# CobayaSampler/cobaya

Measured on AMD Instinct MI355X. Metric: log-posterior evals/sec (whole node), 30-dim gaussian_mixture, higher is better.
Workload: dtype f64

## Files before the change

cobaya_amd/csrc/capi.hip:

```cpp
#include "ctx.h"
#include "host_linalg.h"

int block_slots(const mcmc_hip_ctx* h, int which)
{
    if (!h->blocked) return h->d;
    int L = 0;
    for (size_t b = 0; b < h->blk_size.size(); ++b) {
        if (which == 0) L += h->blk_over[b] * h->blk_size[b];
        else if (which == 1) L += ((int)b <= h->drag_last_slow) ? h->blk_size[b] : 0;
        else L += ((int)b > h->drag_last_slow) ? h->blk_size[b] : 0;
    }
    return L;
}

int upload_constants(mcmc_hip_ctx* h)
{
    if (!h->have_prior || !h->have_target) return MCMC_HIP_OK;
    const int d = h->d, K = h->K;
    const ConstLayout cl{d, K};
    std::vector<double> c((size_t)cl.size() + 16, 0.0);
    for (int i = 0; i < d; ++i) {
        c[cl.lo() + i] = h->lo[i];
        c[cl.hi() + i] = h->hi[i];
        c[cl.loc() + i] = h->loc[i];
// ... 86 lines not shown
        return fail(h, MCMC_HIP_ERR_ARG,
                    "the step kernel needs %zu bytes of LDS per workgroup (> 160 KiB): fewer "
                    "mixture modes or a smaller group_size are required", lds);
    return MCMC_HIP_OK;
}

int set_target_common(mcmc_hip_ctx* h, int K, const double* means, const double* covs,
                      const double* weights, bool normalized)
{
    const int d = h->d;
    if (K < 1 || K > mcmc::kMaxModes)
        return fail(h, MCMC_HIP_ERR_ARG, "n_modes must be in 1..%d, got %d", mcmc::kMaxModes, K);
    if (h->huge && K > mcmc::kHugeMaxModes)
        return fail(h, MCMC_HIP_ERR_ARG, "d=%d > %d serves at most %d mixture modes, got %d", d, kMaxDimBig,
                    mcmc::kHugeMaxModes, K);
    std::vector<double> L((size_t)d * d), Li((size_t)d * d);
    h->mean.assign(means, means + (size_t)K * d);
    h->Linv.assign((size_t)K * d * d, 0.0);
    h->cnorm.assign(K, 0.0);
    h->weight.assign(K, 1.0 / K);
    for (int k = 0; k < K; ++k) {
        const double* C = covs + (size_t)k * d * d;
        if (!is_symmetric(d, C) || !cholesky_lower(d, C, L.data()))
            return fail(h, MCMC_HIP_ERR_NOT_PD,
                        "covariance of mode %d is not a symmetric positive-definite matrix", k);
        tri_inverse_lower(d, L.data(), Li.data());
        std::copy(Li.begin(), Li.end(), h->Linv.begin() + (size_t)k * d * d);
        double logdet = 0.0;
        for (int i = 0; i < d; ++i) logdet += std::log(L[i * d + i]);
        logdet *= 2.0;
        h->cnorm[k] = normalized ? d * std::log(2.0 * M_PI) + logdet : 0.0;
    }
    if (weights) {
        double s = 0.0;
        for (int k = 0; k < K; ++k) {
            if (!(weights[k] >= 0.0)) return fail(h, MCMC_HIP_ERR_ARG, "negative mixture weight");
            s += weights[k];
        }
        if (!(s > 0.0)) return fail(h, MCMC_HIP_ERR_ARG, "mixture weights sum to zero");
        const bool renorm = !(std::fabs(s - 1.0) <= 1e-8 + 1e-5);
        for (int k = 0; k < K; ++k) h->weight[k] = renorm ? weights[k] / s : weights[k];
    }
    h->K = K;
    h->bg.on = false;
    h->fnt.on = false;
    h->have_target = true;
    ++h->dir_epoch;
    h->have_state = false;
    int rc = lds_check(h);
    if (rc) return rc;
    return upload_constants(h);
}

}

extern "C" {

const char* mcmc_hip_version(void) { return "mcmc_hip 0.1 (gfx950)"; }

const char* mcmc_hip_last_error(const mcmc_hip_ctx* h)
{
    return h ? h->err.c_str() : g_create_error.c_str();
}

int mcmc_hip_dim_supported(int d)
{
    return kernels_for_dim(d) != nullptr || big_for_dim(d) != nullptr;
}

int32_t mcmc_hip_max_dim(void) { return mcmc::kMaxDimHuge; }

int mcmc_hip_create(const mcmc_hip_config* cfg, mcmc_hip_ctx** out)
{
    if (!cfg || !out) return fail(nullptr, MCMC_HIP_ERR_ARG, "null argument");
    *out = nullptr;
    if (cfg->d < 1) return fail(nullptr, MCMC_HIP_ERR_ARG, "d must be >= 1, got %d", cfg->d);
    const DimKernels* k = kernels_for_dim(cfg->d);
    const BigKernels* kb = k ? nullptr : big_for_dim(cfg->d);
    const bool huge = cfg->d > kMaxDimBig;
    if (huge) {
        if (cfg->d > mcmc::kMaxDimHuge)
            return fail(nullptr, MCMC_HIP_ERR_ARG, "d=%d is above the largest dimension served (%d)",
                        cfg->d, mcmc::kMaxDimHuge);
        if (!(cfg->flags & MCMC_HIP_FLAG_INCREMENTAL))
            return fail(nullptr, MCMC_HIP_ERR_ARG,
                        "d=%d > %d is served with incremental evaluation only (evaluation: full is not)",
                        cfg->d, kMaxDimBig);
        if (cfg->flags & MCMC_HIP_FLAG_OWN_BASIS)
            return fail(nullptr, MCMC_HIP_ERR_ARG, "d=%d > %d needs the shared basis (shared_basis: False is not served)",
                        cfg->d, kMaxDimBig);
        if (cfg->emit_capacity > 0)
            return fail(nullptr, MCMC_HIP_ERR_ARG,
                        "d=%d > %d emits no rows on the device (emit: chains is not served; use emit: snapshots)",
                        cfg->d, kMaxDimBig);
    }
    if (!k && !kb && !huge)
        return fail(nullptr, MCMC_HIP_ERR_ARG,
                    "no kernels compiled for d=%d (this build covers d = 1..32 lane-per-walker "
                    "and 33..%d column-sweep, as selected at build time)", cfg->d, kMaxDimBig);
    if (cfg->group_size != 64 && cfg->group_size != 128 && cfg->group_size != 256)
        return fail(nullptr, MCMC_HIP_ERR_ARG, "group_size must be 64, 128 or 256, got %d",
                    cfg->group_size);
    if (cfg->n_walkers < cfg->group_size || cfg->n_walkers % cfg->group_size)
        return fail(nullptr, MCMC_HIP_ERR_ARG,
                    "n_walkers (%d) must be a positive multiple of group_size (%d)",
                    cfg->n_walkers, cfg->group_size);
// ... 25 lines not shown
    int ndev = 0;
    hipError_t e = hipGetDeviceCount(&ndev);
    if (e != hipSuccess || ndev <= 0)
        return fail(nullptr, MCMC_HIP_ERR_DEVICE, "no HIP device available (%s)",
                    e == hipSuccess ? "device count 0" : hipGetErrorString(e));
    if (cfg->device < 0 || cfg->device >= ndev)
        return fail(nullptr, MCMC_HIP_ERR_ARG, "device %d out of range (0..%d)", cfg->device,
                    ndev - 1);
    hipDeviceProp_t prop;
    if (hipGetDeviceProperties(&prop, cfg->device) != hipSuccess)
        return fail(nullptr, MCMC_HIP_ERR_DEVICE, "hipGetDeviceProperties failed");
    if (std::strncmp(prop.gcnArchName, "gfx950", 6) != 0)
        return fail(nullptr, MCMC_HIP_ERR_DEVICE,
                    "device %d is %s; this library is built for gfx950 only", cfg->device,
                    prop.gcnArchName);
    if (hipSetDevice(cfg->device) != hipSuccess)
        return fail(nullptr, MCMC_HIP_ERR_DEVICE, "hipSetDevice(%d) failed", cfg->device);
    mcmc_hip_ctx* h = new mcmc_hip_ctx();
    h->cfg = *cfg;
    h->k = k;
    h->kb = kb;
    h->huge = huge;
    h->kp = (kb && !getenv("MCMC_HIP_NO_PAIR_BIG")) ? pair_for_dim(cfg->d) : nullptr;
    h->d = cfg->d;
    h->W = cfg->n_walkers;
    h->gs = cfg->group_size;
    h->G = h->W / h->gs;
    h->bgs = h->gs << ((cfg->flags & MCMC_HIP_FLAG_BASIS_GROUP_MASK) >> 8);
    h->BG = h->W / h->bgs;
    h->shift.assign(h->d, 0.0);
    h->incremental = (cfg->flags & MCMC_HIP_FLAG_INCREMENTAL) != 0;
    h->own_basis = (cfg->flags & MCMC_HIP_FLAG_OWN_BASIS) != 0 && cfg->d > 1;
    if (hipStreamCreateWithFlags(&h->stream, hipStreamNonBlocking) != hipSuccess) {
        delete h;
        return fail(nullptr, MCMC_HIP_ERR_DEVICE, "hipStreamCreate failed");
    }
    const size_t W = h->W, d = h->d, G = h->G, np = d * (d + 1) / 2;
    hipError_t r = hipSuccess;
    auto acc = [&](hipError_t x) { if (r == hipSuccess) r = x; };
    acc(h->x.resize(W * d)); acc(h->logpost.resize(W)); acc(h->logprior.resize(W));
    acc(h->loglike.resize(W)); acc(h->weight_i.resize(W)); acc(h->prej.resize(W));
    acc(h->burn.resize(W)); acc(h->nacc.resize(W)); acc(h->stuck.resize(1));
    acc(h->dT.resize(d * d + 16));  acc(h->Sg.resize(G * np));
    acc(h->gsum.resize(G * d + np + 1));
    if (r == hipSuccess) {
        h->pooled.p = h->gsum.p + G * d;
        h->acc_total.p = reinterpret_cast<unsigned long long*>(h->gsum.p + G * d + np);
    }
    acc(h->dshift.resize(d));
    if (cfg->emit_capacity > 0) {
        acc(h->rows.resize(W * (size_t)cfg->emit_capacity * (d + 4)));
        acc(h->nrows.resize(W));
    }
    acc(hipHostMalloc((void**)&h->pin_mom, sizeof(double) * (G * d + np + 2), hipHostMallocDefault));
    acc(hipHostMalloc((void**)&h->pin_T, sizeof(double) * 4 * d * d, hipHostMallocDefault));
    for (auto& e : h->pin_T_done) acc(hipEventCreateWithFlags(&e, hipEventDisableTiming));
    acc(hipEventCreateWithFlags(&h->mom_event, hipEventDisableTiming));
    if (h->incremental) {
        int prio_least = 0, prio_greatest = 0;
        acc(hipDeviceGetStreamPriorityRange(&prio_least, &prio_greatest));
        acc(hipStreamCreateWithPriority(&h->stream2, hipStreamNonBlocking, prio_least));
        acc(hipEventCreateWithFlags(&h->mark, hipEventDisableTiming));
        acc(hipEventCreateWithFlags(&h->T_event, hipEventDisableTiming));
        if (const char* e = getenv("MCMC_HIP_EAGER_DIRECTIONS")) h->lazy_dirs = !(e[0] && e[0] != '0');
        if (const char* e = getenv("MCMC_HIP_LOOKAHEAD")) h->lookahead = std::max(1, atoi(e));
        if (const char* e = getenv("MCMC_HIP_DUO")) h->duo = (e[0] && e[0] != '0') ? 1 : 0;
        if (const char* e = getenv("MCMC_HIP_ACCEPT_SLACK")) {
            const double v = strtod(e, nullptr);
            h->accept_slack = v < mcmc::kAcceptSlack ? mcmc::kAcceptSlack : v;
        }
        for (auto& D : h->dirs) acc(hipEventCreateWithFlags(&D.ready, hipEventDisableTiming));
        h->prefetch = !getenv("MCMC_HIP_NO_PREFETCH");
    }
    if (r == hipSuccess) r = hipMemsetAsync(h->gsum.p, 0, sizeof(double) * G * d, h->stream);
    if (r == hipSuccess) r = hipMemsetAsync(h->pooled.p, 0, sizeof(double) * np, h->stream);
    if (r == hipSuccess) r = hipMemsetAsync(h->dshift.p, 0, sizeof(double) * d, h->stream);
    if (r == hipSuccess) r = hipMemsetAsync(h->stuck.p, 0, sizeof(int), h->stream);
    if (r == hipSuccess) r = hipMemsetAsync(h->acc_total.p, 0, sizeof(unsigned long long), h->stream);
    if (r == hipSuccess) r = hipStreamSynchronize(h->stream);
    if (r != hipSuccess) {
        fail(nullptr, MCMC_HIP_ERR_DEVICE, "device allocation failed: %s", hipGetErrorString(r));
        mcmc_hip_destroy(h);
        return MCMC_HIP_ERR_DEVICE;
    }
    *out = h;
    return MCMC_HIP_OK;
}

void mcmc_hip_destroy(mcmc_hip_ctx* h)
{
    if (!h) return;
    (void)hipSetDevice(h->cfg.device);
    if (h->stream) (void)hipStreamSynchronize(h->stream);
    if (h->stream2) (void)hipStreamSynchronize(h->stream2);
    resolve_timing(h);
    for (auto e : h->pool) (void)hipEventDestroy(e);
    for (auto& D : h->dirs) {
        D.V.release(); D.Vf.release(); D.VU.release(); D.vflag.release(); D.vflag_f.release(); D.UU.release();
        D.colflag.release(); D.VW.release(); D.NL.release();
        if (D.ready) (void)hipEventDestroy(D.ready);
    }
    if (h->mark) (void)hipEventDestroy(h->mark);
    if (h->T_event) (void)hipEventDestroy(h->T_event);
    if (h->stream2) (void)hipStreamDestroy(h->stream2);
    h->x.release(); h->logpost.release(); h->logprior.release(); h->loglike.release();
    h->hV.release(); h->hScratch.release(); h->hCols.release();
    h->cblock.release(); h->dT.release(); h->V.release(); h->rows.release(); h->gsum.release();
// ... 705 lines not shown
}

int mcmc_hip_read_moments(mcmc_hip_ctx* h, int64_t* n_snapshots, double* group_sum,
                          double* pooled_S, int32_t reset)
{
    if (!h) return MCMC_HIP_ERR_ARG;
    HIP_TRY(h, hipSetDevice(h->cfg.device));
    HIP_TRY(h, hipStreamSynchronize(h->stream));
    if (h->stream2) HIP_TRY(h, hipStreamSynchronize(h->stream2));
    resolve_timing(h);
    const size_t d = h->d, G = h->G, np = d * (d + 1) / 2;
    if (n_snapshots) *n_snapshots = h->n_snapshots;
    if (group_sum)
        HIP_TRY(h, hipMemcpy(group_sum, h->gsum.p, sizeof(double) * G * d, hipMemcpyDeviceToHost));
    if (pooled_S) {
        std::vector<double> p(np);
        HIP_TRY(h, hipMemcpy(p.data(), h->pooled.p, sizeof(double) * np, hipMemcpyDeviceToHost));
        for (size_t i = 0; i < d; ++i)
            for (size_t j = 0; j <= i; ++j)
                pooled_S[i * d + j] = pooled_S[j * d + i] = p[i * (i + 1) / 2 + j];
    }
    if (reset) {
        HIP_TRY(h, hipMemset(h->gsum.p, 0, sizeof(double) * G * d));
        HIP_TRY(h, hipMemset(h->pooled.p, 0, sizeof(double) * np));
        h->n_snapshots = 0;
    }
    return MCMC_HIP_OK;
}

int mcmc_hip_set_moments(mcmc_hip_ctx* h, int64_t n_snapshots, const double* group_sum,
                         const double* pooled_S)
{
    if (!h || !group_sum || !pooled_S || n_snapshots < 0) return MCMC_HIP_ERR_ARG;
    HIP_TRY(h, hipSetDevice(h->cfg.device));
    HIP_TRY(h, hipStreamSynchronize(h->stream));
    const size_t d = h->d, G = h->G, np = d * (d + 1) / 2;
    std::vector<double> p(np);
    for (size_t i = 0; i < d; ++i)
        for (size_t j = 0; j <= i; ++j) p[i * (i + 1) / 2 + j] = pooled_S[i * d + j];
    HIP_TRY(h, hipMemcpy(h->gsum.p, group_sum, sizeof(double) * G * d, hipMemcpyHostToDevice));
    HIP_TRY(h, hipMemcpy(h->pooled.p, p.data(), sizeof(double) * np, hipMemcpyHostToDevice));
    h->n_snapshots = n_snapshots;
    return MCMC_HIP_OK;
}

int mcmc_hip_request_moments(mcmc_hip_ctx* h)
{
    if (!h) return MCMC_HIP_ERR_ARG;
    if (!h->have_state) return fail(h, MCMC_HIP_ERR_STATE, "no state");
    if (h->mom_pending) return fail(h, MCMC_HIP_ERR_STATE, "a moment request is already pending");
    HIP_TRY(h, hipSetDevice(h->cfg.device));
    const size_t d = h->d, G = h->G, np = d * (d + 1) / 2;
    hipStream_t s = h->stream;
    HIP_TRY(h, hipMemcpyAsync(h->pin_mom, h->gsum.p, sizeof(double) * (G * d + np + 1),
                              hipMemcpyDeviceToHost, s));
    HIP_TRY(h, hipMemcpyAsync(h->pin_mom + G * d + np + 1, h->stuck.p, sizeof(int),
                              hipMemcpyDeviceToHost, s));
    if (h->fnt.on)
        HIP_TRY(h, hipMemcpyAsync(reinterpret_cast<int*>(h->pin_mom + G * d + np + 1) + 1, h->fnt.bad.p,
                                  sizeof(int), hipMemcpyDeviceToHost, s));
    h->mom_fn = h->fnt.on;
    if (!h->ck.ring.p) HIP_TRY(h, hipMemsetAsync(h->gsum.p, 0, sizeof(double) * (G * d + np), s));
    HIP_TRY(h, hipEventRecord(h->mom_event, s));
    h->mom_n = h->n_snapshots;
    h->mom_step = h->step;
    h->n_snapshots = 0;
    h->mom_pending = true;
    return MCMC_HIP_OK;
}

int mcmc_hip_fetch_moments(mcmc_hip_ctx* h, int64_t* n_snapshots, double* group_sum,
                           double* pooled_S, int64_t counters[2])
{
    if (!h) return MCMC_HIP_ERR_ARG;
    if (!h->mom_pending) return fail(h, MCMC_HIP_ERR_STATE, "no moment request is pending");
    HIP_TRY(h, hipSetDevice(h->cfg.device));
    HIP_TRY(h, hipEventSynchronize(h->mom_event));
    h->mom_pending = false;
    const size_t d = h->d, G = h->G, np = d * (d + 1) / 2;
    if (n_snapshots) *n_snapshots = h->mom_n;
    if (group_sum) std::copy(h->pin_mom, h->pin_mom + G * d, group_sum);
    if (pooled_S) {
        const double* p = h->pin_mom + G * d;
        for (size_t i = 0; i < d; ++i)
            for (size_t j = 0; j <= i; ++j)
                pooled_S[i * d + j] = pooled_S[j * d + i] = p[i * (i + 1) / 2 + j];
    }
    if (counters) {
        unsigned long long tot;
        std::memcpy(&tot, h->pin_mom + G * d + np, sizeof tot);
        counters[0] = (int64_t)h->mom_step;
        counters[1] = (int64_t)tot;
    }
    if (h->mom_fn) {
        int bad = 0;
        std::memcpy(&bad, reinterpret_cast<const int*>(h->pin_mom + G * d + np + 1) + 1, sizeof bad);
        if (bad) return function_target_error(h, bad);
    }
    int stuck = 0;
    std::memcpy(&stuck, h->pin_mom + G * d + np + 1, sizeof stuck);
    if (stuck)
        return fail(h, MCMC_HIP_ERR_STUCK,
                    "The chain has been stuck for %g attempts (walker %d), stopping sampling.",
                    h->cfg.max_tries, stuck - 1);
    return MCMC_HIP_OK;
}

void mcmc_hip_note_step_kernel(const char* name) { g_noted_kernel = name; }

const char* mcmc_hip_last_step_kernel(const mcmc_hip_ctx* h)
{
    return h ? h->last_step_kernel.c_str() : "";
}

int mcmc_hip_enable_timing(mcmc_hip_ctx* h, int32_t on)
// ... 42 lines not shown
```

cobaya_amd/csrc/ctx.h:

```cpp
#pragma once
#include "../../include/mcmc_hip.h"

#include <algorithm>
#include <cmath>
#include <cstdarg>
#include <cstdio>
#include <cstring>
#include <limits>
#include <string>
#include <vector>

#define MCMC_HIP_HOST_SIDE 1
#include "kernels.h"
#include "huge_args.h"
#include "pliklite_args.h"
#include "function_args.h"
#include "checkpoint_args.h"
#include "marginal_args.h"
#include "autocorr_args.h"
#include "bestfit_args.h"
#include "evidence_args.h"
#include "derived_args.h"
#include "comm.h"
#include "inc_choice.h"
// ... 103 lines not shown
    unsigned long long hV_cycle = ~0ull, hV_epoch = ~0ull;
    hipStream_t stream = nullptr;
    std::string err;
    int d = 0, W = 0, G = 0, gs = 0, K = -1;
    bool have_prior = false, have_target = false, have_cov = false, have_state = false;
    std::vector<int32_t> kind, periodic;
    std::vector<double> lo, hi, loc, scale, mls;
    double uniform_logp = 0.0;
    uint32_t norm_mask = 0, periodic_mask = 0;
    uint32_t norm_mask4[4] = {0, 0, 0, 0};
    bool any_periodic = false;
    std::vector<double> mean, Linv, cnorm, weight;
    std::vector<double> cov, T;
    bool blocked = false;
    std::vector<int32_t> blk_size, blk_over, i_of_j;
    int drag_last_slow = -1, drag_steps = 0;
    DevBuf<int> dblk, vflag, vflag_f;
    DevBuf<double> Vf;
    DevBuf<double> drag_cs;
    std::vector<double> shift;
    DevBuf<double> x, logpost, logprior, loglike, cblock, dT, V, rows, gsum, Sg, pooled, dshift;
    DevBuf<double> ex, elp, ell, eder, escratch, dLrow, dLcol;
    bool incremental = false;
    bool y_valid = false;
    bool own_basis = false;
    int bgs = 0, BG = 0;
    DevBuf<double> y, inc_prior, inc_Lrow, inc_mean;
    DevBuf<double> amode;
    bool amode_valid = false;
    struct DirSet {
        DevBuf<double> V, Vf, VU;
        DevBuf<int> vflag, vflag_f, colflag;
        bool has_flags = false;
        DevBuf<double> UU;
        DevBuf<double> VW, NL;
        hipEvent_t ready = nullptr;
        bool ahead = false;
        unsigned long long step0 = ~0ull, epoch = 0;
        int n = 0;
    } dirs[2];
    int dir_cur = 0;
    unsigned long long dir_epoch = 0;
    hipStream_t stream2 = nullptr;
    hipEvent_t mark = nullptr;
    bool mark_valid = false;
    bool prefetch = true;
    bool lazy_dirs = true;
    int lookahead = 4;
    int duo = -1;
    double accept_slack = mcmc::kAcceptSlack;
    hipEvent_t T_event = nullptr;
    bool T_fresh = false;
    double* pin_mom = nullptr;
    double* pin_T = nullptr;
    int pin_T_slot = 0;
    hipEvent_t pin_T_done[4] = {nullptr, nullptr, nullptr, nullptr};
    hipEvent_t mom_event = nullptr;
    bool mom_pending = false;
    bool mom_fn = false;
    int64_t mom_n = 0;
    unsigned long long mom_step = 0;
    struct HostSlot { double* p = nullptr; size_t cap_rows = 0; };
    std::vector<HostSlot> slots = std::vector<HostSlot>(4);
    int slot_next = 0;
    DevBuf<double> pack_out;
    DevBuf<long long> pack_off;
    DevBuf<int> weight_i, prej, burn, stuck, nrows;
    DevBuf<int> thin_acc;
    int emit_thin = 1;
    DevBuf<long long> nacc;
    DevBuf<unsigned long long> acc_total;
    unsigned long long step = 0;
    int64_t n_snapshots = 0;
    bool timing = false;
    struct Ev {
        hipEvent_t a, b;
        int kind;
    };
    std::vector<Ev> pending;
    std::vector<hipEvent_t> pool;
    double ms[6] = {0, 0, 0, 0, 0, 0};
    int64_t n_seen[6] = {0, 0, 0, 0, 0, 0}, n_timed[6] = {0, 0, 0, 0, 0, 0};
    int64_t n_step_launches = 0;
    std::string last_step_kernel;
    struct Ckpt {
        DevBuf<double> ring, wsum, payload, ws, out;
        DevBuf<unsigned long long> acc_prev;
        int cap = 0;
        long long n_done = 0;
        double* pin_out = nullptr;
        hipEvent_t ev = nullptr;
        bool begun = false, pending = false;
        bool payload_only = false;
    } ck;
    struct Bounds {
        DevBuf<double> ring, bounds, payload;
        int n_slots = 0;
        double* pin = nullptr;
    } bd;
    struct Marginals {
        DevBuf<unsigned long long> slab;
        DevBuf<mcmc::MargEntry> entries;
        unsigned long long* pin = nullptr;
        size_t n_counters = 0, off_pairs = 0;
        int n1 = 0, n2 = 0, bins1 = 0, bins2 = 0, n_entries = 0, lds_words = 0;
        int64_t n_acc = 0;
// ... 177 lines not shown
```

cobaya_amd/csrc/incremental_kernels.hip:

```cpp
#include <string>

#include "incremental_common.h"

#ifndef MCMC_INC_DMA_HIDDEN
#define MCMC_INC_DMA_HIDDEN(dq, mode) ((dq) >= 25 && (mode) == 0)
#endif

namespace mcmc {
namespace {

__host__ __device__ constexpr bool inc_one_wave_regs(int dq, int mode, bool per)
{
    return !per && ((mode == 1 && dq >= 31) || (mode == 2 && dq >= 32));
}

__host__ __device__ constexpr int inc_min_waves(int dq, int mode, bool per = false)
{
    if (per) return MCMC_EXP_WAVES(STEP, dq <= 8 ? 4 : dq <= 31 ? 2 : 1);
    return MCMC_EXP_WAVES(STEP,
        mode == 0 ? (dq <= 12 ? 4 : dq <= 30 ? 2 : 1)
        : mode == 1 ? ((dq <= 8 || dq == 13) ? 4 : dq <= 30 ? 2 : 1)
        : (dq <= 8 ? 4 : dq <= 31 ? 2 : 1));
}

// ... 812 lines not shown
                            const pair_t p = col2[4 * kk];
                            const double delta = ra * p.x;
                            cs[kk] = cs[kk] + delta;
                            ce[kk] = ce[kk] + delta;
                            ys[kk] = fma(ra, p.y, ys[kk]);
                            ye[kk] = fma(ra, p.y, ye[kk]);
                        }
                        cs_lt = sel(acc_m, ps_lt, cs_lt);
                        ce_lp = sel(acc_m, pe_lp, ce_lp);
                        ce_ll = sel(acc_m, pe_ll, ce_ll);
                        ce_lt = sel(acc_m, pe_lt, ce_lt);
                        start_acc += cs_lt;
                        end_acc += ce_lt;
                    }
                }
            }
            const unsigned long long accept_m =
                ~lanes(dead) & metropolis(end_acc / navg, start_acc / navg, Ea0);
            const bool accept = __builtin_amdgcn_inverse_ballot_w64(accept_m);
            const int lim = burn > 0 ? lim10 : lim1;
            burn -= (accept & (burn > 0)) ? 1 : 0;
            lpri = sel(accept_m, ce_lp, lpri);
            llik = sel(accept_m, ce_ll, llik);
            lpost = sel(accept_m, ce_lt, lpost);
            prej = sel(accept_m, 0, prej);
            wt = sel(accept_m, 1, wt + 1);
            nacc += sel(accept_m, 1, 0);
            if (!accept & !dead & (wt - prej > lim) && c == 0) atomicCAS(s.stuck, 0, 1 + (int)gid);
#pragma unroll
            for (int kk = 0; kk < DQ; ++kk) {
                x0[kk] = sel(accept_m, ce[kk], x0[kk]);
                y0[kk] = sel(accept_m, ye[kk], y0[kk]);
            }
        }
        asm volatile("s_waitcnt vmcnt(0)" ::: "memory");
        __syncthreads();
    }
#pragma unroll
    for (int kk = 0; kk < DQ; ++kk) {
        const int i = 4 * kk + c;
        if (i < d) {
            s.x[(size_t)i * W + w] = x0[kk];
            a.y[(size_t)i * W + w] = y0[kk];
        }
    }
    if (c == 0) {
        s.logpost[w] = lpost; s.logprior[w] = lpri; s.loglike[w] = llik;
        s.weight[w] = wt; s.prior_rej[w] = prej; s.burn_left[w] = burn;
        s.n_accept[w] = nacc;
    }
    wave_add_accepts(s.accept_total, (c == 0) ? nacc - nacc0 : 0);
}

__global__ void __launch_bounds__(256) whiten_state_kernel(const double* __restrict__ x,
                                                           double* __restrict__ y,
                                                           const double* __restrict__ mean,
                                                           const double* __restrict__ Lrow, int d,
                                                           int W, int K)
{
    extern __shared__ __attribute__((aligned(16))) double sdev[];
    const int l = threadIdx.x & 63, part = __builtin_amdgcn_readfirstlane(threadIdx.x >> 6),
              w = blockIdx.x * 64 + l;
    const bool live = w < W;
    const int nblk = (d + 3) / 4;
    for (int k = 0; k < K; ++k) {
        __syncthreads();
        if (live)
            for (int i = part; i < d; i += 4) sdev[i * 64 + l] = x[(size_t)i * W + w] - mean[k * d + i];
        __syncthreads();
        if (!live) continue;
        for (int rb = part; rb < nblk; rb += 4) {
            const int j0 = 4 * rb;
            if (j0 + 4 <= d) {
                const double* __restrict__ r0 = Lrow + ((size_t)k * d + j0) * d;
                const double* __restrict__ r1 = r0 + d;
                const double* __restrict__ r2 = r1 + d;
                const double* __restrict__ r3 = r2 + d;
                double a0 = 0.0, a1 = 0.0, a2 = 0.0, a3 = 0.0;
                for (int i = 0; i <= j0; ++i) {
                    const double dv = sdev[i * 64 + l];
                    a0 = fma(r0[i], dv, a0);
                    a1 = fma(r1[i], dv, a1);
                    a2 = fma(r2[i], dv, a2);
                    a3 = fma(r3[i], dv, a3);
                }
                const double d1 = sdev[(j0 + 1) * 64 + l], d2 = sdev[(j0 + 2) * 64 + l],
                             d3 = sdev[(j0 + 3) * 64 + l];
                a1 = fma(r1[j0 + 1], d1, a1);
                a2 = fma(r2[j0 + 1], d1, a2);
                a3 = fma(r3[j0 + 1], d1, a3);
                a2 = fma(r2[j0 + 2], d2, a2);
                a3 = fma(r3[j0 + 2], d2, a3);
                a3 = fma(r3[j0 + 3], d3, a3);
                double* __restrict__ out = y + ((size_t)k * d + j0) * W + w;
                out[0] = a0; out[(size_t)W] = a1; out[2 * (size_t)W] = a2; out[3 * (size_t)W] = a3;
            } else {
                for (int j = j0; j < d; ++j) {
                    const double* __restrict__ row = Lrow + ((size_t)k * d + j) * d;
                    double acc = 0.0;
                    for (int i = 0; i <= j; ++i) acc = fma(row[i], sdev[i * 64 + l], acc);
                    y[((size_t)k * d + j) * W + w] = acc;
                }
            }
        }
    }
}

__global__ void __launch_bounds__(256) whiten_directions_kernel(const IncDirArgs a)
{
    extern __shared__ __attribute__((aligned(16))) double sv[];
    const int l = threadIdx.x & 63, part = __builtin_amdgcn_readfirstlane(threadIdx.x >> 6);
    const int sr = blockIdx.x * 64 + l;
    const int g = blockIdx.y;
    const int d = a.d;
    const bool live = sr < a.n_steps;
    int flag1d = 0;
    if (live) {
        const unsigned long long step = a.step0 + (unsigned long long)sr;
        const int cyc = (int)(step / (unsigned long long)a.cps - a.cycle0);
        const int col = (int)(step % (unsigned long long)a.cps);
        const double* __restrict__ v = a.V + ((size_t)g * a.ncyc + cyc) * a.slab + (size_t)col * a.ld;
        for (int i = part; i < d; i += 4) sv[i * 64 + l] = v[i];
        if (a.vflag) flag1d = a.vflag[((size_t)g * a.ncyc + cyc) * a.cps + col];
    }
    __syncthreads();
    if (!live) return;
    const size_t ocol = a.out_div ? (size_t)(sr / a.out_div) * a.out_cols + a.out_slot0 + sr % a.out_div
                                  : (size_t)sr;
    double2* __restrict__ out = (double2*)a.VU + ((size_t)g * a.out_total + ocol) * (4 * a.dq);
    if (a.colflag && part == 0) a.colflag[(size_t)g * a.out_total + ocol] = flag1d;
    const int nblk = (d + 3) / 4;
    for (int rb = part; rb < nblk; rb += 4) {
        const int j = 4 * rb;
        if (j + 4 <= d) {
            const cdoubles r0 = (cdoubles)(unsigned long long)(a.Lrow + (size_t)j * d);
            const cdoubles r1 = r0 + d;
            const cdoubles r2 = r1 + d;
            const cdoubles r3 = r2 + d;
            double a0 = 0.0, a1 = 0.0, a2 = 0.0, a3 = 0.0;
            for (int i = 0; i <= j; ++i) {
                const double v = sv[i * 64 + l];
                a0 = fma(r0[i], v, a0);
                a1 = fma(r1[i], v, a1);
                a2 = fma(r2[i], v, a2);
                a3 = fma(r3[i], v, a3);
            }
            const double v1 = sv[(j + 1) * 64 + l], v2 = sv[(j + 2) * 64 + l], v3 = sv[(j + 3) * 64 + l];
            a1 = fma(r1[j + 1], v1, a1);
            a2 = fma(r2[j + 1], v1, a2);
            a3 = fma(r3[j + 1], v1, a3);
            a2 = fma(r2[j + 2], v2, a2);
            a3 = fma(r3[j + 2], v2, a3);
            a3 = fma(r3[j + 3], v3, a3);
            out[j] = make_double2(sv[j * 64 + l], a0);
            out[j + 1] = make_double2(v1, a1);
            out[j + 2] = make_double2(v2, a2);
            out[j + 3] = make_double2(v3, a3);
        } else {
            for (int jj = j; jj < d; ++jj) {
                const cdoubles row = (cdoubles)(unsigned long long)(a.Lrow + (size_t)jj * d);
                double acc = 0.0;
                for (int i = 0; i <= jj; ++i) acc = fma(row[i], sv[i * 64 + l], acc);
                out[jj] = make_double2(sv[jj * 64 + l], acc);
            }
        }
    }
    if (part == 3)
        for (int j = d; j < 4 * a.dq; ++j) out[j] = make_double2(0.0, 0.0);
    if (a.UU) {
        __shared__ double sq[4][64];
        __syncthreads();
        double sp = 0.0;
        for (int j = part; j < d; j += 4) {
            const double u = out[j].y;
            sp = fma(u, u, sp);
        }
        sq[part][l] = sp;
        __syncthreads();
        if (part == 0)
            a.UU[(size_t)g * a.out_total + ocol] = (sq[0][l] + sq[1][l]) + (sq[2][l] + sq[3][l]);
    }
    if (a.VW) {
        __shared__ double sn[2][4][64];
        const int dpad = 4 * a.dq;
        const cdoubles pr = (cdoubles)(unsigned long long)a.prior;
        double* __restrict__ wout = a.VW + ((size_t)g * a.out_total + ocol) * dpad;
        double nn = 0.0, lw = 0.0;
        for (int j = part; j < dpad; j += 4) {
            double w = 0.0;
            if (j < d) {
                const double inv = pr[3 * dpad + j], v = sv[j * 64 + l];
                w = (v * inv) * inv;
                nn = fma(v, w, nn);
                lw = fma(pr[2 * dpad + j], w, lw);
            }
            wout[j] = w;
        }
        sn[0][part][l] = nn;
        sn[1][part][l] = lw;
        __syncthreads();
        if (part == 0) {
            double2* __restrict__ nl = (double2*)a.NL + ((size_t)g * a.out_total + ocol);
            *nl = make_double2((sn[0][0][l] + sn[0][1][l]) + (sn[0][2][l] + sn[0][3][l]),
                               (sn[1][0][l] + sn[1][1][l]) + (sn[1][2][l] + sn[1][3][l]));
        }
    }
}

__global__ void __launch_bounds__(64) whiten_directions_mix_kernel(const IncDirArgs a)
{
    extern __shared__ __attribute__((aligned(16))) double sv[];
    const int l = threadIdx.x;
    const int sr = blockIdx.x * 64 + l;
    const int g = blockIdx.y;
    const int d = a.d, K = a.n_modes, dpad = 4 * a.dq;
    const bool live = sr < a.n_steps;
    if (live) {
        const unsigned long long step = a.step0 + (unsigned long long)sr;
        const int cyc = (int)(step / (unsigned long long)a.cps - a.cycle0);
// ... 659 lines not shown
```

cobaya_amd/csrc/walker_kernels.hip:

```cpp
#include "det_math.h"
#include "kernels.h"

#ifndef MCMC_CH
#define MCMC_CH 16
#endif
#ifndef MCMC_D
#error "compile with -DMCMC_D=<dimension>"
#endif

namespace mcmc {
namespace {

constexpr int D = MCMC_D;
constexpr int NPAIR = D * (D + 1) / 2;
constexpr bool kBigD = D > kMaxDimLane;
constexpr int LDV = kBigD ? v_ld(D) : D;

typedef const double __attribute__((address_space(4))) * cptr;
__device__ __forceinline__ cptr as_const(const double* p) { return (cptr)(unsigned long long)p; }
__device__ __forceinline__ cptr launder(cptr p)
{
    unsigned long long v = (unsigned long long)p;
    asm volatile("; operand base of this step" : "+s"(v));
    return (cptr)v;
// ... 1078 lines not shown
    if (l == D - 1) Dmine = (((D - 1) & 1) ? -1.0 : 1.0) * dprod;
    __syncthreads();
    if (l < D) {
#pragma unroll
        for (int k = 0; k < D; ++k) sR[half][l * LDH + k] = Dmine * H[k];
    }
    __syncthreads();
    double Rc[D];
    if (l < D) {
#pragma unroll
        for (int k = 0; k < D; ++k) Rc[k] = sR[half][k * LDH + l];
    }
    __syncthreads();
    if (l < D) {
#pragma unroll
        for (int i = 0; i < D; ++i) {
            double s = 0.0;
#pragma unroll
            for (int k = 0; k <= i; ++k) s = fma(cT[i * D + k], Rc[k], s);
            sR[half][l * LDH + i] = s;
        }
    }
    __syncthreads();
    if (valid) {
        const double* __restrict__ sV = sR[half];
        for (int j = l; j < D * D; j += 32) {
            const int c = j / D, i = j - c * D;
            Vout[j] = sV[c * LDH + i];
        }
    }
}

template <bool MULTI, bool DERIVED>
__global__ void __launch_bounds__(64) evaluate_kernel(const EvalArgs a)
{
    extern __shared__ __attribute__((aligned(16))) double sA[];
    const ConstLayout cl{D, a.n_modes};
    const cptr C = as_const(a.cblock);
    const int tid = threadIdx.x;
    const int p = blockIdx.x * 64 + tid;
    if (p >= a.n) return;
    double t[D];
#pragma unroll
    for (int i = 0; i < D; ++i) t[i] = a.x[(size_t)p * D + i];
    bool inb;
    double lp, ll;
    double* der = DERIVED ? a.derived + (size_t)p * (cl.K > 0 ? cl.K : 1) * D : nullptr;
    eval_point<MULTI, DERIVED, true>(t, C, cl, a.norm_mask, a.uniform_logp, sA + tid, 64, inb, lp,
                                     ll, der);
    a.logprior[p] = inb ? lp : -INFINITY;
    a.loglike[p] = inb ? ll : -INFINITY;
}

__global__ void __launch_bounds__(256) group_moments_kernel(const MomentArgs a)
{
    extern __shared__ __attribute__((aligned(16))) double sX[];
    constexpr int LDX = D | 1;
    const int tid = threadIdx.x, gs = blockDim.x, g = blockIdx.x;
    const int w = g * gs + tid;
#pragma unroll
    for (int i = 0; i < D; ++i) sX[tid * LDX + i] = a.x[(size_t)i * a.W + w] - a.shift[i];
    __syncthreads();
    auto pair_of = [](int p, int& i, int& j) {
        i = (int)((sqrtf(8.0f * (float)p + 1.0f) - 1.0f) * 0.5f);
        while ((i + 1) * (i + 2) / 2 <= p) ++i;
        while (i * (i + 1) / 2 > p) --i;
        j = p - i * (i + 1) / 2;
    };
    const bool sums_ride = NPAIR + D <= 2 * gs;
    for (int p0 = tid; p0 < NPAIR || (sums_ride && p0 < gs); p0 += 2 * gs) {
        const int p1 = p0 + gs;
        const bool has0 = p0 < NPAIR, has1 = p1 < NPAIR;
        const int sidx = tid - (gs - D);
        const bool sum1 = sums_ride && !has1 && p0 < gs && sidx >= 0 && sidx < D;
        int i0 = 0, j0 = 0, i1 = 0, j1 = 0;
        if (has0) pair_of(p0, i0, j0);
        if (has1) pair_of(p1, i1, j1);
        if (sum1) i1 = sidx;
        double s0 = 0.0, s1 = 0.0;
        int l = 0;
        for (; l + 8 <= gs; l += 8) {
            double a0[8], b0[8], a1[8], b1[8];
#pragma unroll
            for (int q = 0; q < 8; ++q) {
                a0[q] = sX[(l + q) * LDX + i0]; b0[q] = sX[(l + q) * LDX + j0];
                a1[q] = sX[(l + q) * LDX + i1]; b1[q] = sX[(l + q) * LDX + j1];
            }
#pragma unroll
            for (int q = 0; q < 8; ++q) {
                s0 = fma(a0[q], b0[q], s0);
                s1 = sum1 ? s1 + a1[q] : fma(a1[q], b1[q], s1);
            }
        }
        for (; l < gs; ++l) {
            s0 = fma(sX[l * LDX + i0], sX[l * LDX + j0], s0);
            s1 = sum1 ? s1 + sX[l * LDX + i1] : fma(sX[l * LDX + i1], sX[l * LDX + j1], s1);
        }
        if (has0) a.Sg[(size_t)g * NPAIR + p0] = s0;
        if (has1) a.Sg[(size_t)g * NPAIR + p1] = s1;
        if (sum1) a.group_sum[(size_t)g * D + sidx] += s1;
    }
    if (!sums_ride && tid < D) {
        double s = 0.0;
        for (int l = 0; l < gs; ++l) s = s + sX[l * LDX + tid];
        a.group_sum[(size_t)g * D + tid] += s;
    }
}

__global__ void __launch_bounds__(64) pool_moments_kernel(const MomentArgs a)
{
    const int p = blockIdx.x * 64 + threadIdx.x;
    if (p >= NPAIR) return;
    double acc = a.pooled[p];
    int g = 0;
    for (; g + 64 <= a.G; g += 64) {
        double v[64];
#pragma unroll
        for (int u = 0; u < 64; ++u) v[u] = a.Sg[(size_t)(g + u) * NPAIR + p];
#pragma unroll
        for (int u = 0; u < 64; ++u) acc += v[u];
    }
    for (; g + 16 <= a.G; g += 16) {
        double v[16];
#pragma unroll
        for (int u = 0; u < 16; ++u) v[u] = a.Sg[(size_t)(g + u) * NPAIR + p];
#pragma unroll
        for (int u = 0; u < 16; ++u) acc += v[u];
    }
    for (; g < a.G; ++g) acc += a.Sg[(size_t)g * NPAIR + p];
    a.pooled[p] = acc;
}

#endif
constexpr size_t kLdsMax = 160 * 1024;
size_t pair_lds(const StepArgs& a)
{
    return sizeof(double) * (size_t)(2 * (256 / a.group_size) * a.slab +
        2 * ((a.norm_mask | a.norm_mask_hi) != 0u ? PairGeom<true>::xf : PairGeom<false>::xf) * 256);
}
bool pair_fits(const StepArgs& a)
{
    if (D >= 55 && (a.norm_mask | a.norm_mask_hi) != 0u) return false;
    return kPair && a.periodic_mask == 0u && a.n_modes == 1 && a.rows == nullptr &&
           a.vflag == nullptr && a.W % 256 == 0 && 256 % a.group_size == 0 &&
           pair_lds(a) <= kLdsMax;
}
hipError_t launch_pair(const StepArgs& a, hipStream_t st)
{
    const bool normp = (a.norm_mask | a.norm_mask_hi) != 0u;
    size_t plds = pair_lds(a);
    const int nwg = a.W / 256;
    const int per_cu = (nwg + 255) / 256;
    size_t want = ((size_t)(160 * 1024) / (size_t)per_cu / 1024) * 1024;
    if (per_cu == 1) want = 96 * 1024;
    if (want > plds) plds = want;
    const bool unit_t = a.temperature == 1.0;
    typedef void (*kern_t)(const StepArgs);
    const kern_t kern = normp ? (unit_t ? step_pair_kernel<true, true> : step_pair_kernel<false, true>)
// ... 42 lines not shown
                                        : "mcmc::step_kernel<false, true, own basis>");
        if (multi) hipLaunchKernelGGL((step_kernel<true, true, true>), grid, block, own_lds, st, a);
        else hipLaunchKernelGGL((step_kernel<false, true, true>), grid, block, own_lds, st, a);
        return hipGetLastError();
    }
    if (lds > kLdsMax) return hipErrorInvalidValue;
    if (pair_fits(a)) return launch_pair(a, st);
    const void* fn = multi ? (general ? (const void*)step_kernel<true, true>
                                      : (const void*)step_kernel<true, false>)
                           : (general ? (const void*)step_kernel<false, true>
                                      : (const void*)step_kernel<false, false>);
    if (lds > 64 * 1024) {
        hipError_t e = hipFuncSetAttribute(fn, hipFuncAttributeMaxDynamicSharedMemorySize, (int)lds);
        if (e != hipSuccess) return e;
    }
    mcmc_hip_note_step_kernel(multi ? (general ? "mcmc::step_kernel<true, true>"
                                               : "mcmc::step_kernel<true, false>")
                                    : (general ? "mcmc::step_kernel<false, true>"
                                               : "mcmc::step_kernel<false, false>"));
    if (multi) {
        if (general) hipLaunchKernelGGL((step_kernel<true, true>), grid, block, lds, st, a);
        else hipLaunchKernelGGL((step_kernel<true, false>), grid, block, lds, st, a);
    } else {
        if (general) hipLaunchKernelGGL((step_kernel<false, true>), grid, block, lds, st, a);
        else hipLaunchKernelGGL((step_kernel<false, false>), grid, block, lds, st, a);
    }
    return hipGetLastError();
}

hipError_t launch_basis(const BasisArgs& a, int n_groups, hipStream_t st)
{
    const int n_problems = n_groups * a.ncyc;
    hipLaunchKernelGGL(basis_kernel, dim3((n_problems + 1) / 2), dim3(64), 0, st, a, n_problems);
    return hipGetLastError();
}

hipError_t launch_evaluate(const EvalArgs& a, hipStream_t st)
{
    const bool multi = a.n_modes > 1;
    const size_t lds = sizeof(double) * (size_t)(multi ? a.n_modes * 64 : 0);
    const dim3 grid((a.n + 63) / 64), block(64);
    if (multi) {
        if (a.derived) hipLaunchKernelGGL((evaluate_kernel<true, true>), grid, block, lds, st, a);
        else hipLaunchKernelGGL((evaluate_kernel<true, false>), grid, block, lds, st, a);
    } else {
        if (a.derived) hipLaunchKernelGGL((evaluate_kernel<false, true>), grid, block, lds, st, a);
        else hipLaunchKernelGGL((evaluate_kernel<false, false>), grid, block, lds, st, a);
    }
    return hipGetLastError();
}

hipError_t launch_moments(const MomentArgs& a, int group_size, hipStream_t st)
{
    const size_t lds = sizeof(double) * (size_t)group_size * (D | 1);
    hipLaunchKernelGGL(group_moments_kernel, dim3(a.G), dim3(group_size), lds, st, a);
    hipLaunchKernelGGL(pool_moments_kernel, dim3((NPAIR + 63) / 64), dim3(64), 0, st, a);
    return hipGetLastError();
}

hipError_t launch_drag(const DragArgs& a, hipStream_t st)
{
    const bool multi = a.s.n_modes > 1;
    const int bs = (a.s.W % 256 == 0) ? 256 : 64;
    const size_t lds = sizeof(double) * bs * (size_t)(2 * D + (multi ? a.s.n_modes : 0));
    const dim3 grid(a.s.W / bs), block(bs);
    if (lds > 64 * 1024) {
        hipError_t e = hipFuncSetAttribute(multi ? (const void*)drag_kernel<true> : (const void*)drag_kernel<false>,
                                           hipFuncAttributeMaxDynamicSharedMemorySize, (int)lds);
        if (e != hipSuccess) return e;
    }
    mcmc_hip_note_step_kernel(multi ? "mcmc::drag_kernel<true>" : "mcmc::drag_kernel<false>");
    if (multi) hipLaunchKernelGGL(drag_kernel<true>, grid, block, lds, st, a);
    else hipLaunchKernelGGL(drag_kernel<false>, grid, block, lds, st, a);
    return hipGetLastError();
}

const DimKernels kKernels = {launch_step, launch_basis, launch_evaluate, launch_moments,
                             launch_drag};
#else
const PairKernels kPairKernels = {pair_fits, launch_pair};
#endif

}
}

#define MCMC_CAT2(a, b) a##b
#define MCMC_CAT(a, b) MCMC_CAT2(a, b)
#if MCMC_D <= 32
extern "C" const mcmc::DimKernels* MCMC_CAT(mcmc_hip_dim_, MCMC_D)() { return &mcmc::kKernels; }
#else
static_assert(MCMC_D <= mcmc::kMaxDimPair, "two-wave kernel: d <= kMaxDimPair");
extern "C" const mcmc::PairKernels* MCMC_CAT(mcmc_hip_pair_, MCMC_D)() { return &mcmc::kPairKernels; }
#endif
```

Measured before the change: 90.23 billion.

## Tile moment kernel 2x2, share triangular matvec helper, fuse moment readout kernel

The group moments kernel now computes 2x2 tiles of the covariance from double2 rows in LDS, with register double-buffering, in place of one pair per thread. Whitening and direction-update kernels share a new triangular row-block matvec helper. It 8-way unrolls the inner loops, pairs light and heavy row blocks to balance the triangle, and batches global loads. The moment readout becomes a single kernel that writes into mapped coherent host memory and zeroes the accumulators, replacing several memcpys and a memset. The costs are more code, new group_size restrictions, and device writes over PCIe to host memory.

```diff
diff --git a/cobaya_amd/csrc/capi.hip b/cobaya_amd/csrc/capi.hip
--- a/cobaya_amd/csrc/capi.hip
+++ b/cobaya_amd/csrc/capi.hip
@@ -162,6 +162,26 @@
     return upload_constants(h);
 }
 
+}
+
+namespace mcmc {
+namespace {
+__global__ void __launch_bounds__(256) readout_moments_kernel(unsigned long long* __restrict__ acc,
+                                                              size_t n_acc, const int* __restrict__ stuck,
+                                                              const int* __restrict__ fn_bad,
+                                                              unsigned long long* __restrict__ pin, int zero)
+{
+    const size_t i = (size_t)blockIdx.x * 256 + threadIdx.x;
+    if (i < n_acc) {
+        pin[i] = acc[i];
+        if (zero) acc[i] = 0ull;
+    } else if (i == n_acc) {
+        pin[i] = acc[i];
+        const unsigned lo = (unsigned)*stuck, hi = fn_bad ? (unsigned)*fn_bad : 0u;
+        pin[i + 1] = (unsigned long long)lo | ((unsigned long long)hi << 32);
+    }
+}
+}
 }
 
 extern "C" {
@@ -293,7 +313,9 @@
         acc(h->rows.resize(W * (size_t)cfg->emit_capacity * (d + 4)));
         acc(h->nrows.resize(W));
     }
-    acc(hipHostMalloc((void**)&h->pin_mom, sizeof(double) * (G * d + np + 2), hipHostMallocDefault));
+    acc(hipHostMalloc((void**)&h->pin_mom, sizeof(double) * (G * d + np + 2),
+                      hipHostMallocCoherent | hipHostMallocMapped));
+    if (h->pin_mom) acc(hipHostGetDevicePointer((void**)&h->pin_mom_dev, h->pin_mom, 0));
     acc(hipHostMalloc((void**)&h->pin_T, sizeof(double) * 4 * d * d, hipHostMallocDefault));
     for (auto& e : h->pin_T_done) acc(hipEventCreateWithFlags(&e, hipEventDisableTiming));
     acc(hipEventCreateWithFlags(&h->mom_event, hipEventDisableTiming));
@@ -1105,15 +1127,15 @@
     HIP_TRY(h, hipSetDevice(h->cfg.device));
     const size_t d = h->d, G = h->G, np = d * (d + 1) / 2;
     hipStream_t s = h->stream;
-    HIP_TRY(h, hipMemcpyAsync(h->pin_mom, h->gsum.p, sizeof(double) * (G * d + np + 1),
-                              hipMemcpyDeviceToHost, s));
-    HIP_TRY(h, hipMemcpyAsync(h->pin_mom + G * d + np + 1, h->stuck.p, sizeof(int),
-                              hipMemcpyDeviceToHost, s));
-    if (h->fnt.on)
-        HIP_TRY(h, hipMemcpyAsync(reinterpret_cast<int*>(h->pin_mom + G * d + np + 1) + 1, h->fnt.bad.p,
-                                  sizeof(int), hipMemcpyDeviceToHost, s));
+    {
+        const size_t n_acc = G * d + np;
+        hipLaunchKernelGGL(mcmc::readout_moments_kernel, dim3((unsigned)((n_acc + 1 + 255) / 256)),
+                           dim3(256), 0, s, reinterpret_cast<unsigned long long*>(h->gsum.p), n_acc,
+                           (const int*)h->stuck.p, h->fnt.on ? (const int*)h->fnt.bad.p : nullptr,
+                           h->pin_mom_dev, h->ck.ring.p ? 0 : 1);
+        HIP_TRY(h, hipGetLastError());
+    }
     h->mom_fn = h->fnt.on;
-    if (!h->ck.ring.p) HIP_TRY(h, hipMemsetAsync(h->gsum.p, 0, sizeof(double) * (G * d + np), s));
     HIP_TRY(h, hipEventRecord(h->mom_event, s));
     h->mom_n = h->n_snapshots;
     h->mom_step = h->step;
diff --git a/cobaya_amd/csrc/ctx.h b/cobaya_amd/csrc/ctx.h
--- a/cobaya_amd/csrc/ctx.h
+++ b/cobaya_amd/csrc/ctx.h
@@ -179,6 +179,7 @@
     hipEvent_t T_event = nullptr;
     bool T_fresh = false;
     double* pin_mom = nullptr;
+    unsigned long long* pin_mom_dev = nullptr;
     double* pin_T = nullptr;
     int pin_T_slot = 0;
     hipEvent_t pin_T_done[4] = {nullptr, nullptr, nullptr, nullptr};
diff --git a/cobaya_amd/csrc/incremental_kernels.hip b/cobaya_amd/csrc/incremental_kernels.hip
--- a/cobaya_amd/csrc/incremental_kernels.hip
+++ b/cobaya_amd/csrc/incremental_kernels.hip
@@ -888,6 +888,84 @@
     wave_add_accepts(s.accept_total, (c == 0) ? nacc - nacc0 : 0);
 }
 
+template <int NR>
+__device__ __forceinline__ void rows_times_column(cdoubles L, int d, int j0,
+                                                  const double* __restrict__ col, double (&acc)[NR])
+{
+    cdoubles r[NR];
+#pragma unroll
+    for (int q = 0; q < NR; ++q) { r[q] = L + (size_t)(j0 + q) * d; acc[q] = 0.0; }
+    int i = 0;
+    for (; i + 8 <= j0; i += 8) {
+        double c[8], m[NR][8];
+#pragma unroll
+        for (int u = 0; u < 8; ++u) {
+            c[u] = col[(i + u) * 64];
+#pragma unroll
+            for (int q = 0; q < NR; ++q) m[q][u] = r[q][i + u];
+        }
+#pragma unroll
+        for (int u = 0; u < 8; ++u)
+#pragma unroll
+            for (int q = 0; q < NR; ++q) acc[q] = fma(m[q][u], c[u], acc[q]);
+    }
+    if (i < j0) {
+        double c[4], m[NR][4];
+#pragma unroll
+        for (int u = 0; u < 4; ++u) {
+            c[u] = col[(i + u) * 64];
+#pragma unroll
+            for (int q = 0; q < NR; ++q) m[q][u] = r[q][i + u];
+        }
+#pragma unroll
+        for (int u = 0; u < 4; ++u)
+#pragma unroll
+            for (int q = 0; q < NR; ++q) acc[q] = fma(m[q][u], c[u], acc[q]);
+    }
+    double c[NR], m[NR][NR];
+#pragma unroll
+    for (int u = 0; u < NR; ++u) {
+        c[u] = col[(j0 + u) * 64];
+#pragma unroll
+        for (int q = u; q < NR; ++q) m[q][u] = r[q][j0 + u];
+    }
+#pragma unroll
+    for (int u = 0; u < NR; ++u)
+#pragma unroll
+        for (int q = u; q < NR; ++q) acc[q] = fma(m[q][u], c[u], acc[q]);
+}
+
+template <class Put>
+__device__ __forceinline__ void row_blocks_times_column(cdoubles L, int d, int part,
+                                                        const double* __restrict__ col, Put&& put)
+{
+    const int nblk = (d + 3) / 4;
+    for (int pr = part; 2 * pr < nblk; pr += 4) {
+        for (int s = 0; s < 2; ++s) {
+            const int rb = s ? nblk - 1 - pr : pr;
+            if (s && rb == pr) break;
+            const int j0 = 4 * rb, nr = d - j0;
+            if (nr >= 4) {
+                double acc[4];
+                rows_times_column<4>(L, d, j0, col, acc);
+                put(j0, acc[0]); put(j0 + 1, acc[1]); put(j0 + 2, acc[2]); put(j0 + 3, acc[3]);
+            } else if (nr == 3) {
+                double acc[3];
+                rows_times_column<3>(L, d, j0, col, acc);
+                put(j0, acc[0]); put(j0 + 1, acc[1]); put(j0 + 2, acc[2]);
+            } else if (nr == 2) {
+                double acc[2];
+                rows_times_column<2>(L, d, j0, col, acc);
+                put(j0, acc[0]); put(j0 + 1, acc[1]);
+            } else {
+                double acc[1];
+                rows_times_column<1>(L, d, j0, col, acc);
+                put(j0, acc[0]);
+            }
+        }
+    }
+}
+
 __global__ void __launch_bounds__(256) whiten_state_kernel(const double* __restrict__ x,
                                                            double* __restrict__ y,
                                                            const double* __restrict__ mean,
@@ -898,47 +976,29 @@
     const int l = threadIdx.x & 63, part = __builtin_amdgcn_readfirstlane(threadIdx.x >> 6),
               w = blockIdx.x * 64 + l;
     const bool live = w < W;
-    const int nblk = (d + 3) / 4;
     for (int k = 0; k < K; ++k) {
         __syncthreads();
-        if (live)
-            for (int i = part; i < d; i += 4) sdev[i * 64 + l] = x[(size_t)i * W + w] - mean[k * d + i];
+        if (live) {
+            for (int i0 = part; i0 < d; i0 += 32) {
+                double xv[8];
+#pragma unroll
+                for (int u = 0; u < 8; ++u) {
+                    const int i = i0 + 4 * u;
+                    xv[u] = i < d ? x[(size_t)i * W + w] : 0.0;
+                }
+#pragma unroll
+                for (int u = 0; u < 8; ++u) {
+                    const int i = i0 + 4 * u;
+                    if (i < d) sdev[i * 64 + l] = xv[u] - mean[k * d + i];
+                }
+            }
+        }
         __syncthreads();
         if (!live) continue;
-        for (int rb = part; rb < nblk; rb += 4) {
-            const int j0 = 4 * rb;
-            if (j0 + 4 <= d) {
-                const double* __restrict__ r0 = Lrow + ((size_t)k * d + j0) * d;
-                const double* __restrict__ r1 = r0 + d;
-                const double* __restrict__ r2 = r1 + d;
-                const double* __restrict__ r3 = r2 + d;
-                double a0 = 0.0, a1 = 0.0, a2 = 0.0, a3 = 0.0;
-                for (int i = 0; i <= j0; ++i) {
-                    const double dv = sdev[i * 64 + l];
-                    a0 = fma(r0[i], dv, a0);
-                    a1 = fma(r1[i], dv, a1);
-                    a2 = fma(r2[i], dv, a2);
-                    a3 = fma(r3[i], dv, a3);
-                }
-                const double d1 = sdev[(j0 + 1) * 64 + l], d2 = sdev[(j0 + 2) * 64 + l],
-                             d3 = sdev[(j0 + 3) * 64 + l];
-                a1 = fma(r1[j0 + 1], d1, a1);
-                a2 = fma(r2[j0 + 1], d1, a2);
-                a3 = fma(r3[j0 + 1], d1, a3);
-                a2 = fma(r2[j0 + 2], d2, a2);
-                a3 = fma(r3[j0 + 2], d2, a3);
-                a3 = fma(r3[j0 + 3], d3, a3);
-                double* __restrict__ out = y + ((size_t)k * d + j0) * W + w;
-                out[0] = a0; out[(size_t)W] = a1; out[2 * (size_t)W] = a2; out[3 * (size_t)W] = a3;
-            } else {
-                for (int j = j0; j < d; ++j) {
-                    const double* __restrict__ row = Lrow + ((size_t)k * d + j) * d;
-                    double acc = 0.0;
-                    for (int i = 0; i <= j; ++i) acc = fma(row[i], sdev[i * 64 + l], acc);
-                    y[((size_t)k * d + j) * W + w] = acc;
-                }
-            }
-        }
+        const cdoubles L = (cdoubles)(unsigned long long)(Lrow + (size_t)k * d * d);
+        double* __restrict__ out = y + (size_t)k * d * W + w;
+        row_blocks_times_column(L, d, part, sdev + l,
+                                [&](int j, double v) { out[(size_t)j * W] = v; });
     }
 }
 
@@ -956,7 +1016,14 @@
         const int cyc = (int)(step / (unsigned long long)a.cps - a.cycle0);
         const int col = (int)(step % (unsigned long long)a.cps);
         const double* __restrict__ v = a.V + ((size_t)g * a.ncyc + cyc) * a.slab + (size_t)col * a.ld;
-        for (int i = part; i < d; i += 4) sv[i * 64 + l] = v[i];
+        for (int i0 = part; i0 < d; i0 += 32) {
+            double vv[8];
+#pragma unroll
+            for (int u = 0; u < 8; ++u) vv[u] = i0 + 4 * u < d ? v[i0 + 4 * u] : 0.0;
+#pragma unroll
+            for (int u = 0; u < 8; ++u)
+                if (i0 + 4 * u < d) sv[(i0 + 4 * u) * 64 + l] = vv[u];
+        }
         if (a.vflag) flag1d = a.vflag[((size_t)g * a.ncyc + cyc) * a.cps + col];
     }
     __syncthreads();
@@ -965,42 +1032,8 @@
                                   : (size_t)sr;
     double2* __restrict__ out = (double2*)a.VU + ((size_t)g * a.out_total + ocol) * (4 * a.dq);
     if (a.colflag && part == 0) a.colflag[(size_t)g * a.out_total + ocol] = flag1d;
-    const int nblk = (d + 3) / 4;
-    for (int rb = part; rb < nblk; rb += 4) {
-        const int j = 4 * rb;
-        if (j + 4 <= d) {
-            const cdoubles r0 = (cdoubles)(unsigned long long)(a.Lrow + (size_t)j * d);
-            const cdoubles r1 = r0 + d;
-            const cdoubles r2 = r1 + d;
-            const cdoubles r3 = r2 + d;
-            double a0 = 0.0, a1 = 0.0, a2 = 0.0, a3 = 0.0;
-            for (int i = 0; i <= j; ++i) {
-                const double v = sv[i * 64 + l];
-                a0 = fma(r0[i], v, a0);
-                a1 = fma(r1[i], v, a1);
-                a2 = fma(r2[i], v, a2);
-                a3 = fma(r3[i], v, a3);
-            }
-            const double v1 = sv[(j + 1) * 64 + l], v2 = sv[(j + 2) * 64 + l], v3 = sv[(j + 3) * 64 + l];
-            a1 = fma(r1[j + 1], v1, a1);
-            a2 = fma(r2[j + 1], v1, a2);
-            a3 = fma(r3[j + 1], v1, a3);
-            a2 = fma(r2[j + 2], v2, a2);
-            a3 = fma(r3[j + 2], v2, a3);
-            a3 = fma(r3[j + 3], v3, a3);
-            out[j] = make_double2(sv[j * 64 + l], a0);
-            out[j + 1] = make_double2(v1, a1);
-            out[j + 2] = make_double2(v2, a2);
-            out[j + 3] = make_double2(v3, a3);
-        } else {
-            for (int jj = j; jj < d; ++jj) {
-                const cdoubles row = (cdoubles)(unsigned long long)(a.Lrow + (size_t)jj * d);
-                double acc = 0.0;
-                for (int i = 0; i <= jj; ++i) acc = fma(row[i], sv[i * 64 + l], acc);
-                out[jj] = make_double2(sv[jj * 64 + l], acc);
-            }
-        }
-    }
+    row_blocks_times_column((cdoubles)(unsigned long long)a.Lrow, d, part, sv + l,
+                            [&](int j, double u) { out[j] = make_double2(sv[j * 64 + l], u); });
     if (part == 3)
         for (int j = d; j < 4 * a.dq; ++j) out[j] = make_double2(0.0, 0.0);
     if (a.UU) {
diff --git a/cobaya_amd/csrc/walker_kernels.hip b/cobaya_amd/csrc/walker_kernels.hip
--- a/cobaya_amd/csrc/walker_kernels.hip
+++ b/cobaya_amd/csrc/walker_kernels.hip
@@ -1154,58 +1154,84 @@
     a.loglike[p] = inb ? ll : -INFINITY;
 }
 
+constexpr int kMomNb = (D + 1) / 2;
+constexpr int kMomLd = (2 * kMomNb) % 4 == 2 ? 2 * kMomNb : 2 * kMomNb + 2;
+constexpr int kMomTiles = kMomNb * (kMomNb + 1) / 2;
+
 __global__ void __launch_bounds__(256) group_moments_kernel(const MomentArgs a)
 {
     extern __shared__ __attribute__((aligned(16))) double sX[];
-    constexpr int LDX = D | 1;
     const int tid = threadIdx.x, gs = blockDim.x, g = blockIdx.x;
     const int w = g * gs + tid;
-#pragma unroll
-    for (int i = 0; i < D; ++i) sX[tid * LDX + i] = a.x[(size_t)i * a.W + w] - a.shift[i];
+    {
+        double xv[2 * kMomNb];
+#pragma unroll
+        for (int i = 0; i < 2 * kMomNb; ++i) xv[i] = i < D ? a.x[(size_t)i * a.W + w] : 0.0;
+        double2* __restrict__ row = (double2*)(sX + tid * kMomLd);
+#pragma unroll
+        for (int k = 0; k < kMomNb; ++k)
+            row[k] = make_double2(xv[2 * k] - a.shift[2 * k],
+                                  2 * k + 1 < D ? xv[2 * k + 1] - a.shift[2 * k + 1] : 0.0);
+    }
     __syncthreads();
-    auto pair_of = [](int p, int& i, int& j) {
-        i = (int)((sqrtf(8.0f * (float)p + 1.0f) - 1.0f) * 0.5f);
-        while ((i + 1) * (i + 2) / 2 <= p) ++i;
-        while (i * (i + 1) / 2 > p) --i;
-        j = p - i * (i + 1) / 2;
-    };
-    const bool sums_ride = NPAIR + D <= 2 * gs;
-    for (int p0 = tid; p0 < NPAIR || (sums_ride && p0 < gs); p0 += 2 * gs) {
-        const int p1 = p0 + gs;
-        const bool has0 = p0 < NPAIR, has1 = p1 < NPAIR;
-        const int sidx = tid - (gs - D);
-        const bool sum1 = sums_ride && !has1 && p0 < gs && sidx >= 0 && sidx < D;
-        int i0 = 0, j0 = 0, i1 = 0, j1 = 0;
-        if (has0) pair_of(p0, i0, j0);
-        if (has1) pair_of(p1, i1, j1);
-        if (sum1) i1 = sidx;
-        double s0 = 0.0, s1 = 0.0;
-        int l = 0;
-        for (; l + 8 <= gs; l += 8) {
-            double a0[8], b0[8], a1[8], b1[8];
-#pragma unroll
-            for (int q = 0; q < 8; ++q) {
-                a0[q] = sX[(l + q) * LDX + i0]; b0[q] = sX[(l + q) * LDX + j0];
-                a1[q] = sX[(l + q) * LDX + i1]; b1[q] = sX[(l + q) * LDX + j1];
-            }
-#pragma unroll
-            for (int q = 0; q < 8; ++q) {
-                s0 = fma(a0[q], b0[q], s0);
-                s1 = sum1 ? s1 + a1[q] : fma(a1[q], b1[q], s1);
-            }
-        }
-        for (; l < gs; ++l) {
-            s0 = fma(sX[l * LDX + i0], sX[l * LDX + j0], s0);
-            s1 = sum1 ? s1 + sX[l * LDX + i1] : fma(sX[l * LDX + i1], sX[l * LDX + j1], s1);
-        }
-        if (has0) a.Sg[(size_t)g * NPAIR + p0] = s0;
-        if (has1) a.Sg[(size_t)g * NPAIR + p1] = s1;
-        if (sum1) a.group_sum[(size_t)g * D + sidx] += s1;
-    }
-    if (!sums_ride && tid < D) {
-        double s = 0.0;
-        for (int l = 0; l < gs; ++l) s = s + sX[l * LDX + tid];
-        a.group_sum[(size_t)g * D + tid] += s;
+    constexpr int B = 8;
+    for (int t = tid; t < kMomTiles; t += gs) {
+        int I = (int)((sqrtf(8.0f * (float)t + 1.0f) - 1.0f) * 0.5f);
+        while ((I + 1) * (I + 2) / 2 <= t) ++I;
+        while (I * (I + 1) / 2 > t) --I;
+        const int J = t - I * (I + 1) / 2;
+        const double2* __restrict__ pa = (const double2*)(sX + 2 * I);
+        const double2* __restrict__ pb = (const double2*)(sX + 2 * J);
+        double s00 = 0.0, s01 = 0.0, s10 = 0.0, s11 = 0.0;
+        double2 A[2][B], Bv[2][B];
+#pragma unroll
+        for (int q = 0; q < B; ++q) {
+            A[0][q] = pa[q * (kMomLd / 2)];
+            Bv[0][q] = pb[q * (kMomLd / 2)];
+        }
+        for (int l = 0; l < gs; l += 2 * B) {
+#pragma unroll
+            for (int h = 0; h < 2; ++h) {
+                const int nxt = l + (h + 1) * B;
+                if (nxt < gs) {
+#pragma unroll
+                    for (int q = 0; q < B; ++q) {
+                        A[h ^ 1][q] = pa[(nxt + q) * (kMomLd / 2)];
+                        Bv[h ^ 1][q] = pb[(nxt + q) * (kMomLd / 2)];
+                    }
+                }
+#pragma unroll
+                for (int q = 0; q < B; ++q) {
+                    s00 = fma(A[h][q].x, Bv[h][q].x, s00);
+                    s01 = fma(A[h][q].x, Bv[h][q].y, s01);
+                    s10 = fma(A[h][q].y, Bv[h][q].x, s10);
+                    s11 = fma(A[h][q].y, Bv[h][q].y, s11);
+                }
+            }
+        }
+        double* __restrict__ Sg = a.Sg + (size_t)g * NPAIR;
+        const int i0 = 2 * I, j0 = 2 * J, i1 = i0 + 1, j1 = j0 + 1;
+        Sg[i0 * (i0 + 1) / 2 + j0] = s00;
+        if (I != J) Sg[i0 * (i0 + 1) / 2 + j1] = s01;
+        if (i1 < D) {
+            Sg[i1 * (i1 + 1) / 2 + j0] = s10;
+            if (j1 < D) Sg[i1 * (i1 + 1) / 2 + j1] = s11;
+        }
+    }
+    if ((tid >> 6) == (gs >> 6) - 1) {
+        for (int k = tid & 63; k < kMomNb; k += 64) {
+            const double2* __restrict__ pa = (const double2*)(sX + 2 * k);
+            double s0 = 0.0, s1 = 0.0;
+            for (int l = 0; l < gs; l += B) {
+                double2 v[B];
+#pragma unroll
+                for (int q = 0; q < B; ++q) v[q] = pa[(l + q) * (kMomLd / 2)];
+#pragma unroll
+                for (int q = 0; q < B; ++q) { s0 = s0 + v[q].x; s1 = s1 + v[q].y; }
+            }
+            a.group_sum[(size_t)g * D + 2 * k] += s0;
+            if (2 * k + 1 < D) a.group_sum[(size_t)g * D + 2 * k + 1] += s1;
+        }
     }
 }
 
@@ -1354,7 +1380,9 @@
 
 hipError_t launch_moments(const MomentArgs& a, int group_size, hipStream_t st)
 {
-    const size_t lds = sizeof(double) * (size_t)group_size * (D | 1);
+    if (group_size <= 0 || group_size > 256 || group_size % 64 != 0)
+        return hipErrorInvalidValue;
+    const size_t lds = sizeof(double) * (size_t)group_size * kMomLd;
     hipLaunchKernelGGL(group_moments_kernel, dim3(a.G), dim3(group_size), lds, st, a);
     hipLaunchKernelGGL(pool_moments_kernel, dim3((NPAIR + 63) / 64), dim3(64), 0, st, a);
     return hipGetLastError();
```

Result: faster. 91.42 billion, median of 6 (+1.3%).
